# nh273/caro-ai

Measured on AMD Instinct MI355X. Metric: self-play MCTS node-expansions/sec/GPU (Connect4, 200 sims/move); 1->8 GPU scaling, higher is better.
Workload: dtype f32

## Files before the change

caro_ai_amd/_lib.py:

```python
import ctypes as C
import os

_HERE = os.path.dirname(os.path.abspath(__file__))
LIB_PATH = os.path.join(_HERE, "libcaro_hip.so")
if os.environ.get("CARO_HIP_LIB"):
    LIB_PATH = os.environ["CARO_HIP_LIB"]

GAME_CONNECT4, GAME_MNK, GAME_CARO = 0, 1, 2
RESIGNED = -2


class CaroError(RuntimeError):
    pass


class CaroConfig(C.Structure):
    _fields_ = [
        ("game_kind", C.c_int32), ("n", C.c_int32), ("k", C.c_int32), ("n_games", C.c_int32),
        ("n_stores", C.c_int32), ("n_nets", C.c_int32), ("max_batch", C.c_int32), ("node_cap", C.c_int32),
        ("steps_before_tau_0", C.c_int32), ("first_player_mode", C.c_int32),
        ("c_puct", C.c_float), ("alpha", C.c_double), ("explore", C.c_double),
        ("seed", C.c_uint64), ("uid_base", C.c_uint64), ("uid_stride", C.c_uint64),
        ("device_id", C.c_int32), ("evict", C.c_int32), ("stagger", C.c_int32), ("stagger_recycle", C.c_int32),
        ("games_limit", C.c_int64),
# ... 73 lines not shown
    "caro_stream_destroy": (C.c_int, [_P]),
    "caro_search_batch": (C.c_int, [_P, _P, _P, C.c_int, C.c_int, _P, _P, _P, _P, _P, _P]),
    "caro_search_move": (C.c_int, [_P, _P, _P, C.c_int, C.c_int] + [_P] * 10),
    "caro_net_forward_pair": (C.c_int, [_P, _P, _P, _P, C.c_int64, _P, _P, _P]),
    "caro_net_forward_pair_at": (C.c_int, [_P, _P, _P, _P, C.c_int64, C.c_int64, _P, _P, _P]),
    "caro_net_forward_slots": (C.c_int, [_P, _P, _P, _P, _P, C.c_int, C.c_int, _P, _P, _P]),
    "caro_net_forward_slot_list": (C.c_int, [_P, _P, _P, _P, _P, _P, C.c_int, C.c_int, _P, _P, _P]),
    "caro_net_create_hash": (C.c_int, [C.c_int, C.c_int, C.c_int, C.c_uint64, C.c_int, _P]),
    "caro_net_create_hash_grain": (C.c_int, [C.c_int, C.c_int, C.c_int, C.c_uint64, C.c_int, C.c_int, _P]),
    "caro_net_forward_stamped": (C.c_int, [_P, _P, _P, C.c_int, C.c_int64, _P, _P, _P, _P]),
    "caro_net_debug_stamps": (C.c_int, [_P, _P]),
    "caro_get_descent": (C.c_int, [_P, C.c_int, C.c_int, _P, _P, _P, _P, _P, _P]),
    "caro_select_cancel": (C.c_int, [_P]),
    "caro_expand_backup": (C.c_int, [_P, _P, _P, _P]),
    "caro_policy": (C.c_int, [_P, _P, _P, _P]),
    "caro_step": (C.c_int, [_P, _P, _P, _P, _P, _P]),
    "caro_drain_tuples": (C.c_int, [_P, C.c_int64, _P, _P, _P, _P, _P, C.c_int, _P, _P, _P]),
    "caro_drain_tuples_begin": (C.c_int, [_P, C.c_int64, _P, _P, _P, _P, _P, C.c_int, _P]),
    "caro_drain_tuples_end": (C.c_int, [_P, _P, _P]),
    "caro_search_staggered": (C.c_int, [_P, _P, _P, C.c_int, C.c_int, _P, _P, _P, _P, _P]),
    "caro_drain_parked_begin": (C.c_int, [_P, C.c_int64, _P, _P, _P, _P, _P, _P]),
    "caro_engine_set_resign": (C.c_int, [_P, C.c_double, C.c_double]),
    "caro_drain_tuples_begin_q": (C.c_int, [_P, C.c_int64, _P, _P, _P, _P, _P, C.c_int, _P, _P]),
    "caro_drain_parked_begin_q": (C.c_int, [_P, C.c_int64, _P, _P, _P, _P, _P, _P, _P]),
    "caro_engine_set_playout_cap": (C.c_int, [_P, C.c_double, C.c_int]),
    "caro_drain_tuples_begin_x": (C.c_int, [_P, C.c_int64, _P, _P, _P, _P, _P, C.c_int, _P, _P, _P]),
    "caro_drain_parked_begin_x": (C.c_int, [_P, C.c_int64, _P, _P, _P, _P, _P, _P, _P, _P]),
    "caro_engine_set_early_stop": (C.c_int, [_P, C.c_int]),
    "caro_engine_set_openings": (C.c_int, [_P, C.c_int]),
    "caro_engine_set_forced_playouts": (C.c_int, [_P, C.c_double]),
    "caro_forced_stats": (C.c_int, [_P, _P, _P]),
    "caro_engine_set_kernel_form": (C.c_int, [_P, C.c_int]),
    "caro_engine_kernel_form": (C.c_int, [_P]),
    "caro_engine_set_fpu": (C.c_int, [_P, C.c_double, C.c_double]),
    "caro_host_fpu_level": (C.c_int, [C.c_int, C.c_int, _P, _P, _P, _P, _P, _P, _P, C.c_float, C.c_double, C.c_float,
                                      C.c_double, _P]),
    "caro_engine_set_virtual_loss": (C.c_int, [_P, C.c_int]),
    "caro_host_vl_level": (C.c_int, [C.c_int, C.c_int, _P, _P, _P, _P, _P, _P, _P, C.c_float, C.c_double, _P, C.c_int, _P]),
    "caro_engine_set_temperature": (C.c_int, [_P, C.c_double, C.c_double, C.c_int]),
    "caro_host_temperature": (C.c_int, [C.c_int, _P, C.c_double, _P]),
    "caro_host_forced_root": (C.c_int, [C.c_int, _P, _P, _P, _P, C.c_double, C.c_double, _P]),
    "caro_host_forced_prune": (C.c_int, [C.c_int, _P, _P, _P, C.c_float, C.c_double, _P]),
    "caro_drain_tuples_begin_ex": (C.c_int, [_P, C.c_int64, _P, _P, _P, _P, _P, C.c_int, C.POINTER(CaroDrainExtra), _P]),
    "caro_drain_parked_begin_ex": (C.c_int, [_P, C.c_int64, _P, _P, _P, _P, _P, C.POINTER(CaroDrainExtra), _P]),
    "caro_pool_open": (C.c_int, [_P, C.c_int64, _P, _P, _P, _P]),
    "caro_pool_set": (C.c_int, [_P, C.c_int64, _P, _P, _P, _P, _P]),
    "caro_pool_select": (C.c_int, [_P, C.c_int64, _P, _P]),
    "caro_pool_hold": (C.c_int, [_P, _P]),
    "caro_pool_level": (C.c_int, [_P, C.c_int64, _P, _P, _P, _P]),
    "caro_pool_select_budget": (C.c_int, [_P, C.c_int64, _P, _P, _P]),
    "caro_principal_lines": (C.c_int, [_P, C.c_int64, _P, C.c_int, C.c_int, C.c_int] + [_P] * 11),
    "caro_host_line_heads": (C.c_int, [C.c_int, _P, C.c_int, _P]),
    "caro_counters": (C.c_int, [_P, _P, _P]),
    "caro_live_games": (C.c_int, [_P, _P, _P]),
    "caro_pending_leaves": (C.c_int, [_P, _P, _P]),
    "caro_debug_stamps": (C.c_int, [_P, C.c_int]),
    "caro_debug_read": (C.c_int, [_P, _P, C.c_int64, _P]),
    "caro_debug_sqrt_check": (C.c_int, [C.c_uint32, _P]),
    "caro_profile_enable": (C.c_int, [_P, C.c_int]),
    "caro_profile_read": (C.c_int, [_P, _P, _P, C.c_int]),
    "caro_profile_begin": (C.c_int, [_P, C.c_int, _P]),
    "caro_profile_end": (None, [_P, C.c_int, _P]),
    "caro_tree_sizes": (C.c_int, [_P, _P, _P]),
    "caro_tree_live": (C.c_int, [_P, _P, _P]),
    "caro_lookup_nodes": (C.c_int, [_P, C.c_int64] + [_P] * 10),
    "caro_get_roots": (C.c_int, [_P] * 6),
# ... 33 lines not shown
```

caro_ai_amd/csrc/caro_engine.hip:

```cpp
#include <hip/hip_runtime.h>

#include <cstddef>
#include <cstdio>
#include <cstdlib>
#include <cstring>
#include <string>
#include <type_traits>
#include <vector>

#include "../../include/caro_hip.h"
#include "../../include/caro_noise.h"
#include "caro_rules.h"
#include "caro_variants.h"

namespace caro {

constexpr uint32_t NSTRONG = 1u << 30;
constexpr uint32_t NMASK = NSTRONG - 1u;
constexpr int ST_DROPPED = 0, ST_TERMINAL = 1, ST_LEAF = 2;
constexpr int MAXB = 64;
constexpr int DONE_HELD = 3;

enum Counter { C_SIMS, C_LEVELS, C_EXPANSIONS, C_TERMINALS, C_DROPPED, C_OVERFLOW, C_PLIES, C_FINISHED, C_N };

// ... 2615 lines not shown
    s_t[tid] += a;
    s_g[tid] += b;
    __syncthreads();
  }
  long long ot = s_t[tid] - ct;
  int og = s_g[tid] - cg;
  __shared__ long long s_tot;
  __shared__ int s_totg;
  if (tid == 0) { s_tot = 0; s_totg = 0; }
  __syncthreads();
  for (int g = lo; g < hi; ++g) {
    int sel = 0;
    if (v.done[g] == 1) {
      if (ot + v.ply[g] <= cap) {
        sel = 1;
        v.dr_off[g] = (int)ot;
        v.dr_gidx[g] = og;
        atomicMax((unsigned long long*)&s_tot, (unsigned long long)(ot + v.ply[g]));
        atomicMax(&s_totg, og + 1);
      }
      ot += v.ply[g];
      og += 1;
    }
    v.dr_sel[g] = sel;
  }
  __syncthreads();
  if (tid == 0) {
    v.dr_tot[0] = s_tot;
    v.dr_tot[1] = s_totg;
  }
}

template <class GEO>
__global__ void k_drain_copy(View v, uint64_t* __restrict__ states, int32_t* __restrict__ players,
                             double* __restrict__ pi, int32_t* __restrict__ z, int64_t* __restrict__ games,
                             double* __restrict__ root_q, uint8_t* __restrict__ full, uint16_t* __restrict__ mbs,
                             int16_t* __restrict__ open, int recycle) {
  constexpr int KW = GEO::KW;
  const int g = blockIdx.x;
  if (!v.dr_sel[g]) return;
  const int n = v.ply[g];
  const int off = v.dr_off[g];
  const int r = v.final_r[g];
  const uint64_t uid0 = v.uid[g];
  const int16_t made0 = open ? v.open_made[g] : (int16_t)0;
  for (int idx = threadIdx.x; idx < n * v.A; idx += blockDim.x) {
    const int j = idx / v.A, a = idx % v.A;
    const int plyi = n - 1 - j;
    pi[((size_t)off + j) * v.A + a] = v.h_pi[((size_t)g * v.maxply + plyi) * v.A + a];
  }
  for (int j = threadIdx.x; j < n; j += blockDim.x) {
    const int plyi = n - 1 - j;
    const size_t hi = (size_t)g * v.maxply + plyi;
    for (int w = 0; w < KW; ++w) states[((size_t)off + j) * KW + w] = v.h_key[hi * KW + w];
    players[off + j] = v.h_player[hi];
    z[off + j] = (j & 1) ? -r : r;
    if (root_q) root_q[off + j] = v.h_q[hi];
    if (full) full[off + j] = v.h_full[hi];
    if (mbs) mbs[off + j] = v.h_mb[hi];
    if (open) open[off + j] = made0;
  }
  if (threadIdx.x == 0 && games) {
    int64_t* rec = games + (size_t)v.dr_gidx[g] * 4;
    rec[0] = (int64_t)uid0;
    rec[1] = v.first[g];
    rec[2] = v.result[g];
    rec[3] = v.step[g];
  }
  __syncthreads();
  if (recycle && game_wanted(v, g, uid0 + v.uid_stride)) {
    reset_game<GEO>(v, g, uid0 + v.uid_stride, -1);
  } else if (threadIdx.x == 0) {
    v.done[g] = 2;
  }
}

__global__ void k_sum_counters(View v) {
  __shared__ unsigned long long s[256];
  for (int c = 0; c < C_N; ++c) {
    unsigned long long acc = 0;
    for (int g = threadIdx.x; g < v.G; g += blockDim.x) acc += v.counters[(size_t)g * C_N + c];
    s[threadIdx.x] = acc;
    __syncthreads();
    for (int d = 128; d > 0; d >>= 1) {
      if (threadIdx.x < d) s[threadIdx.x] += s[threadIdx.x + d];
      __syncthreads();
    }
    if (threadIdx.x == 0) v.counters_sum[c] = s[0];
    __syncthreads();
  }
}

__global__ void k_sum_forced(View v) {
  __shared__ unsigned long long s[256];
  for (int c = 0; c < 4; ++c) {
    unsigned long long acc = 0;
    for (int g = threadIdx.x; g < v.G; g += blockDim.x) acc += v.fp_ctr[(size_t)g * 4 + c];
    s[threadIdx.x] = acc;
    __syncthreads();
    for (int d = 128; d > 0; d >>= 1) {
      if (threadIdx.x < d) s[threadIdx.x] += s[threadIdx.x + d];
      __syncthreads();
    }
    if (threadIdx.x == 0) v.fp_sum[c] = s[0];
    __syncthreads();
  }
// ... 296 lines not shown
__global__ void k_noise(uint64_t seed, long long M, int A, double alpha, const uint64_t* uid, const uint32_t* ply,
                        const uint32_t* sim, double* out) {
  constexpr int LPD = GEO::LPD, APL = GEO::APL;
  const int grp = threadIdx.x / LPD, l = threadIdx.x % LPD;
  const long long m = (long long)blockIdx.x * (blockDim.x / LPD) + grp;
  const long long mm = m < M ? m : M - 1;
  const uint64_t key = caro_noise_key(seed, uid[mm], ply[mm], sim[mm]);
  double nz[APL];
  __shared__ double s_mail[APL > 1 ? 2 * GEO::AP : 1];
  noise_group<LPD, APL>(key, l, A, alpha, nz, s_mail);
  if (m < M)
    for (int j = 0; j < APL; ++j) {
      const int a = l * APL + j;
      if (a < A) out[(size_t)m * A + a] = nz[j];
    }
}

}

using namespace caro;

static thread_local std::string g_err;
static int fail(int code, const std::string& msg) {
  g_err = msg;
  return code;
}
#define HIPCHK(x)                                                                                  \
  do {                                                                                             \
    hipError_t e_ = (x);                                                                           \
    if (e_ != hipSuccess)                                                                          \
      return fail(CARO_E_HIP, std::string(#x) + ": " + hipGetErrorString(e_));                     \
  } while (0)

struct caro_engine {
  caro_config cfg{};
  Variant var = V_BAD;
  View v{};
  std::vector<void*> allocs;
  int32_t* pinned = nullptr;
  int64_t* pinned64 = nullptr;
  int32_t* scratch = nullptr;
  int32_t* live = nullptr;
  int select_pending = 0;
  int drain_pending = 0;
  int ls_mid = 0;
  int ls_forced = 0;
  int stag_batch = 0;
  hipEvent_t drain_ev = nullptr;
  int prof_on = 0;
  int prof_gate = 1;
  uint64_t prof_ctr = 0;
  uint64_t prof_cal = 0;
  int32_t* rows = nullptr;
  int rows_par = 0;
  int fused_ok = 1;
  int force_full = 0;
  int32_t* pool_host = nullptr;
  std::vector<hipEvent_t> ev;
  std::vector<int> ev_kind;
  size_t ev_used = 0;
  double prof_ms[8] = {};
  long long prof_n[8] = {};
};

static bool tree_lean(const caro_engine* h) {
  const View& v = h->v;
  return !h->force_full && !v.q_on && !v.cap_on && !v.es_on && !v.open_made && !v.fp_on && !v.fpu_on && !v.vl_n && !v.temp_on && !v.lv_on && v.n_stores == 1 && !v.dbg;
}
static bool tree_vl(const caro_engine* h, int batch) { return h->v.vl_n > 0 && batch > 1; }
enum TreeForm { FORM_LEAN, FORM_FULL, FORM_VL };
static TreeForm opening_form(const caro_engine* h, int batch, bool one_wave) {
  if (one_wave && tree_lean(h)) return FORM_LEAN;
  return tree_vl(h, batch) ? FORM_VL : FORM_FULL;
}
static TreeForm closing_form(const caro_engine* h, bool one_wave) { return one_wave && tree_lean(h) ? FORM_LEAN : FORM_FULL; }
#define TREE_FORMS3(form, EXPR)                            \
  switch (form) {                                          \
    case FORM_LEAN: { using OPT = TreeLean; EXPR; } break; \
    case FORM_VL: { using OPT = TreeVl; EXPR; } break;     \
    default: { using OPT = TreeFull; EXPR; } break;        \
  }
#define TREE_FORMS2(form, EXPR)                            \
  if ((form) == FORM_VL) { using OPT = TreeVl; EXPR; }     \
  else { using OPT = TreeFull; EXPR; }

enum : unsigned { R_LEVELS = 1, R_STAG = 2, R_SELECT = 4, R_DRAIN = 8 };
static int guard(const caro_engine* h, const char* who, unsigned what,
                 const char* stag_tail = "use caro_search_staggered / caro_drain_parked_begin") {
  const auto no = [who](const char* text, const char* tail = "") { return fail(CARO_E_STATE, std::string(who) + text + tail); };
// ... 233 lines not shown
  int rc = 0;
#define DA(p, n) if ((rc = dalloc(h, &p, (n))) != 0) { caro_engine_destroy(h); return rc; }
  DA(v.tbl, T);
  DA(v.node_key, T * v.ntab * v.tstride * KW);
  DA(v.edges, T * v.etab * v.tstride * 4 * AP);
  DA(v.n_nodes, T);
  DA(v.n_created, T);
  DA(v.root, G * KW);
  DA(v.player, G); DA(v.ply, G); DA(v.step, G); DA(v.uid, G); DA(v.done, G); DA(v.result, G); DA(v.final_r, G);
  DA(v.first, G);
  DA(v.h_key, G * v.maxply * KW);
  DA(v.h_player, G * v.maxply);
  DA(v.h_pi, G * v.maxply * v.A);
  DA(v.path_rec, G * v.maxB * v.maxd);
  DA(v.d_rec, G * v.maxB);
  DA(v.d_key, G * v.maxB * KW);
  DA(v.g_nleaf, G); DA(v.g_off, G); DA(v.g_tree, G); DA(v.g_class, G); DA(v.g_pack, G);
  DA(v.slot_list, 2 * G * v.maxB);
  DA(v.leaf_count, 4);
  DA(v.counters, G * C_N);
  DA(v.counters_sum, C_N);
  DA(v.dr_off, G); DA(v.dr_gidx, G); DA(v.dr_sel, G); DA(v.dr_tot, 2);
  DA(h->scratch, (size_t)v.maxd + 8);
  DA(h->live, 1);
  DA(h->rows, 8);
  if (cfg->stagger > 0) {
    DA(v.lm, G); DA(v.pend, G); DA(v.wait, G); DA(v.dirty, T);
    DA(v.pk_flag, G); DA(v.pk_ply, G); DA(v.pk_final_r, G); DA(v.pk_first, G); DA(v.pk_result, G); DA(v.pk_step, G);
    DA(v.pk_uid, G);
    DA(v.handed, 1);
    DA(v.ph_key, G * v.maxply * KW);
    DA(v.ph_player, G * v.maxply);
    DA(v.ph_pi, G * v.maxply * v.A);
  }
#undef DA
  HIPCHK(hipHostMalloc((void**)&h->pinned, 64, hipHostMallocDefault));
  HIPCHK(hipHostMalloc((void**)&h->pinned64, 128, hipHostMallocDefault));
  *out = h;
  rc = fresh_state(h, nullptr);
  if (rc) { caro_engine_destroy(h); *out = nullptr; return rc; }
  HIPCHK(hipDeviceSynchronize());
  return 0;
}

int caro_engine_restart(caro_engine* h, const caro_config* cfg, void* stream) {
  if (!h || !cfg) return fail(CARO_E_INVAL, "null argument");
  const caro_config& o = h->cfg;
  if (cfg->game_kind != o.game_kind || cfg->n != o.n || cfg->k != o.k || cfg->n_games != o.n_games ||
      cfg->n_stores != o.n_stores || cfg->n_nets != o.n_nets || cfg->max_batch != o.max_batch ||
      cfg->node_cap != o.node_cap || (cfg->evict != 0) != (o.evict != 0) || cfg->device_id != o.device_id ||
      (cfg->stagger > 0) != (o.stagger > 0))
    return fail(CARO_E_INVAL, "caro_engine_restart: the configuration differs from the engine's in a field that shapes its "
                              "memory (game, n_games, n_stores, n_nets, max_batch, node_cap, evict, device, staggered or not)");
  if (cfg->stagger < 0) return fail(CARO_E_INVAL, "stagger must be >= 0");
  if (int rc = guard(h, "caro_engine_restart", R_DRAIN)) return rc;
  if (int rc = guard(h, "caro_engine_restart", R_SELECT)) return rc;
  HIPCHK(hipSetDevice(o.device_id));
  h->cfg = *cfg;
  apply_run_params(h, cfg);
  return fresh_state(h, (hipStream_t)stream);
}

int caro_engine_set_resign(caro_engine* h, double threshold, double playthrough) {
  if (!h) return fail(CARO_E_INVAL, "null engine");
  if (!(threshold >= -1.0 && threshold <= 1.0)) return fail(CARO_E_INVAL, "resign threshold must be in [-1, 1]");
  if (!(playthrough >= 0.0 && playthrough <= 1.0)) return fail(CARO_E_INVAL, "resign playthrough must be in [0, 1]");
  View& v = h->v;
  if (!v.q_on) {
    HIPCHK(hipSetDevice(h->cfg.device_id));
    const size_t n = (size_t)v.G * v.maxply;
// ... 557 lines not shown

int caro_drain_parked_begin(caro_engine* h, int64_t cap, uint64_t* states, int32_t* players, double* pi, int32_t* z,
                            int64_t* games, void* stream) {
  return caro_drain_parked_begin_q(h, cap, states, players, pi, z, games, nullptr, stream);
}
int caro_drain_parked_begin_q(caro_engine* h, int64_t cap, uint64_t* states, int32_t* players, double* pi, int32_t* z,
                              int64_t* games, double* root_q, void* stream) {
  return caro_drain_parked_begin_x(h, cap, states, players, pi, z, games, root_q, nullptr, stream);
}
int caro_drain_parked_begin_x(caro_engine* h, int64_t cap, uint64_t* states, int32_t* players, double* pi, int32_t* z,
                              int64_t* games, double* root_q, uint8_t* full, void* stream) {
  caro_drain_extra ex = {(uint32_t)sizeof(caro_drain_extra), root_q, full, nullptr, nullptr};
  return caro_drain_parked_begin_ex(h, cap, states, players, pi, z, games, &ex, stream);
}
static int drain_extra(const caro_engine* h, const char* who, const caro_drain_extra* in, caro_drain_extra* out) {
  *out = caro_drain_extra{(uint32_t)sizeof(caro_drain_extra), nullptr, nullptr, nullptr, nullptr};
  if (!in) return 0;
  if (in->size < offsetof(caro_drain_extra, root_q_dev)) return fail(CARO_E_INVAL, "caro_drain_extra.size is not set");
  if (in->size >= offsetof(caro_drain_extra, root_q_dev) + sizeof(double*)) out->root_q_dev = in->root_q_dev;
  if (in->size >= offsetof(caro_drain_extra, full_dev) + sizeof(uint8_t*)) out->full_dev = in->full_dev;
  if (in->size >= offsetof(caro_drain_extra, minibatches_dev) + sizeof(uint16_t*)) out->minibatches_dev = in->minibatches_dev;
  if (in->size >= offsetof(caro_drain_extra, open_dev) + sizeof(int16_t*)) out->open_dev = in->open_dev;
  const std::string w(who);
  if (out->open_dev && !h->v.open_made) return fail(CARO_E_STATE, w + "_ex: open_dev before caro_engine_set_openings (no opening counts recorded)");
  if (out->minibatches_dev && !h->v.es_on) return fail(CARO_E_STATE, w + "_ex: minibatches_dev before caro_engine_set_early_stop (no minibatch counts recorded)");
  if (out->root_q_dev && !h->v.q_on) return fail(CARO_E_STATE, w + "_q before caro_engine_set_resign (no root Q recorded)");
  if (out->full_dev && !h->v.cap_on) return fail(CARO_E_STATE, w + "_x before caro_engine_set_playout_cap (no ply classes recorded)");
  return 0;
}
static int drain_rows(caro_engine* h, const char* who, const View& dv, int64_t cap, uint64_t* states, int32_t* players,
                      double* pi, int32_t* z, int64_t* games, const caro_drain_extra& ex, int recycle, hipStream_t st) {
  if (h->drain_pending) return fail(CARO_E_STATE, std::string(who) + " twice without caro_drain_tuples_end");
  if (!h->drain_ev) HIPCHK(hipEventCreateWithFlags(&h->drain_ev, hipEventDisableTiming));
  hipLaunchKernelGGL(k_drain_scan, dim3(1), dim3(1024), 0, st, dv, (long long)cap);
  DISPATCH(h->var, hipLaunchKernelGGL(k_drain_copy<GEO>, dim3(dv.G), dim3(256), 0, st, dv, states, players, pi, z, games,
                                      ex.root_q_dev, ex.full_dev, ex.minibatches_dev, ex.open_dev, recycle));
  return 0;
}
static int drain_totals(caro_engine* h, hipStream_t st) {
  HIPCHK(hipGetLastError());
  HIPCHK(hipMemcpyAsync(h->pinned64 + 8, h->v.dr_tot, 2 * sizeof(int64_t), hipMemcpyDeviceToHost, st));
  HIPCHK(hipEventRecord(h->drain_ev, st));
  h->drain_pending = 1;
  return 0;
}
int caro_drain_parked_begin_ex(caro_engine* h, int64_t cap, uint64_t* states, int32_t* players, double* pi, int32_t* z,
                               int64_t* games, const caro_drain_extra* extra, void* stream) {
  if (!h || !states || !players || !pi || !z) return fail(CARO_E_INVAL, "null argument");
  caro_drain_extra ex;
  if (int rc = drain_extra(h, "caro_drain_parked_begin", extra, &ex)) return rc;
  if (!h->v.stag_S) return fail(CARO_E_STATE, "the engine was not created in staggered mode (caro_config.stagger)");
  hipStream_t st = (hipStream_t)stream;
  View pv = h->v;
  pv.done = h->v.pk_flag; pv.ply = h->v.pk_ply; pv.final_r = h->v.pk_final_r; pv.first = h->v.pk_first;
  pv.result = h->v.pk_result; pv.step = h->v.pk_step; pv.uid = h->v.pk_uid;
  pv.h_key = h->v.ph_key; pv.h_player = h->v.ph_player; pv.h_pi = h->v.ph_pi; pv.h_q = h->v.ph_q;
  pv.h_full = h->v.ph_full;
  pv.h_mb = h->v.ph_mb;
  pv.open_made = h->v.pk_open;
  if (int rc = drain_rows(h, "caro_drain_parked_begin", pv, cap, states, players, pi, z, games, ex, 0, st)) return rc;
  if (h->v.stag_pool)
    DISPATCH(h->var, hipLaunchKernelGGL(k_stag_assign<GEO>, dim3(1), dim3(1024), 0, st, h->v));
  DISPATCH(h->var, hipLaunchKernelGGL(k_stag_clean<GEO>, dim3(h->v.G * h->v.n_stores), dim3(256), 0, st, h->v));
  return drain_totals(h, st);
}

int caro_policy(caro_engine* h, double* pi, int32_t* counts, void* stream) {
  if (!h) return fail(CARO_E_INVAL, "null engine");
  DISPATCH(h->var, hipLaunchKernelGGL(k_policy<GEO>, dim3(h->v.G), dim3(64), 0, (hipStream_t)stream, h->v, pi, counts));
  HIPCHK(hipGetLastError());
  return 0;
}

int caro_step(caro_engine* h, const double* uniforms, int32_t* actions, int32_t* done, int32_t* result, void* stream) {
  if (!h) return fail(CARO_E_INVAL, "null engine");
  if (int rc = guard(h, "caro_step", R_STAG | R_SELECT)) return rc;
  const int p0 = prof_begin(h, PK_STEP, (hipStream_t)stream);
  DISPATCH(h->var, hipLaunchKernelGGL(k_step<GEO>, dim3(h->v.G), dim3(64), 0, (hipStream_t)stream, h->v, uniforms,
                                      actions, done, result));
  prof_end(h, p0, (hipStream_t)stream);
  h->ls_mid = 0;
  h->ls_forced = 0;
  if (h->cfg.evict)
    DISPATCH(h->var, hipLaunchKernelGGL(k_evict<GEO>, dim3(h->v.G), dim3(256), 0, (hipStream_t)stream, h->v));
  HIPCHK(hipGetLastError());
  return 0;
}

int caro_drain_tuples_begin(caro_engine* h, int64_t cap, uint64_t* states, int32_t* players, double* pi, int32_t* z,
                            int64_t* games, int recycle, void* stream) {
  return caro_drain_tuples_begin_q(h, cap, states, players, pi, z, games, recycle, nullptr, stream);
}
// ... 50 lines not shown
  *counts_dev = h->v.leaf_count;
  return 0;
}

int caro_stream_create_partition(int device_id, int part, int nparts, void** stream_out) {
  if (!stream_out || nparts < 1 || part < 0 || part >= nparts) return fail(CARO_E_INVAL, "bad partition");
  HIPCHK(hipSetDevice(device_id));
  hipDeviceProp_t prop;
  HIPCHK(hipGetDeviceProperties(&prop, device_id));
  const int ncu = prop.multiProcessorCount;
  const int words = (ncu + 31) / 32;
  std::vector<uint32_t> mask(words, 0u);
  const int lo = (int)((long long)ncu * part / nparts), hi = (int)((long long)ncu * (part + 1) / nparts);
  for (int c = lo; c < hi; ++c) mask[c >> 5] |= 1u << (c & 31);
  hipStream_t st = nullptr;
  HIPCHK(hipExtStreamCreateWithCUMask(&st, (uint32_t)words, mask.data()));
  *stream_out = (void*)st;
  return 0;
}
int caro_stream_destroy(void* stream) {
  if (stream) HIPCHK(hipStreamDestroy((hipStream_t)stream));
  return 0;
}

int caro_engine_set_kernel_form(caro_engine* h, int form) {
  if (!h) return fail(CARO_E_INVAL, "null engine");
  if (form != 0 && form != 1) return fail(CARO_E_INVAL, "kernel form must be 0 (automatic) or 1 (always the full form)");
  h->force_full = form;
  return 0;
}
int caro_engine_kernel_form(const caro_engine* h) {
  if (!h) return fail(CARO_E_INVAL, "null engine");
  return tree_lean(h) ? 0 : 1;
}

int caro_debug_stamps(caro_engine* h, int on) {
  if (!h) return fail(CARO_E_INVAL, "null engine");
  if (on && !h->v.dbg) {
    void* q = nullptr;
    HIPCHK(hipMalloc(&q, (size_t)h->v.G * 16 * sizeof(unsigned long long)));
    HIPCHK(hipMemset(q, 0, (size_t)h->v.G * 16 * sizeof(unsigned long long)));
    h->allocs.push_back(q);
    h->v.dbg = (unsigned long long*)q;
  } else if (!on) {
    h->v.dbg = nullptr;
  }
  return 0;
}
int caro_debug_read(caro_engine* h, uint64_t* out_host, int64_t n_u64, void* stream) {
  if (!h || !out_host || !h->v.dbg) return fail(CARO_E_INVAL, "no stamp buffer");
  if (n_u64 > (int64_t)h->v.G * 16) n_u64 = (int64_t)h->v.G * 16;
  HIPCHK(hipStreamSynchronize((hipStream_t)stream));
  HIPCHK(hipMemcpy(out_host, h->v.dbg, n_u64 * sizeof(uint64_t), hipMemcpyDeviceToHost));
  return 0;
}

int caro_debug_sqrt_check(uint32_t n_max, uint64_t* bad_host) {
  if (!bad_host || n_max > (1u << 24)) return fail(CARO_E_INVAL, "bad argument");
  unsigned long long* bad = nullptr;
  HIPCHK(hipMalloc(&bad, sizeof(unsigned long long)));
  HIPCHK(hipMemset(bad, 0, sizeof(unsigned long long)));
  hipLaunchKernelGGL(k_sqrt_check, dim3(1024), dim3(256), 0, (hipStream_t) nullptr, n_max, bad);
  HIPCHK(hipGetLastError());
  HIPCHK(hipMemcpy(bad_host, bad, sizeof(unsigned long long), hipMemcpyDeviceToHost));
  HIPCHK(hipFree(bad));
  return 0;
// ... 146 lines not shown
```

caro_ai_amd/engine.py:

```python
import ctypes as C

import numpy as np
import torch

from caro_ai_amd import _lib
from caro_ai_amd import early_stop
from caro_ai_amd import forced_playouts as forced_playouts_mod
from caro_ai_amd import fpu as fpu_mod
from caro_ai_amd import openings as openings_mod
from caro_ai_amd import selfplay_options
from caro_ai_amd import temperature as temperature_mod
from caro_ai_amd import virtual_loss as virtual_loss_mod
from caro_ai_amd import config as cfg

COUNTER_NAMES = ["sims", "levels", "expansions", "terminals", "dropped", "overflows", "plies", "finished"]


HIP_NET_MODES = {"hip": "f32", "hipw": "f32w", "hipw1": "f32w1", "hipw2": "f32w2", "hipx3": "bf16x3"}

def lanes_per_descent(game):
    A = game.action_space
    return 8 if A == 7 else 16 if A <= 16 else 32 if A <= 32 else 64


def staggered_geometry(game, batch, evict=False):
    t = int(batch) * lanes_per_descent(game)
    return t >= 64 and t % 64 == 0 and (t > 64 or not evict)


def _ptr(t):
    return C.c_void_p(t.data_ptr()) if t is not None else None


def torch_evaluator(net, form="gemm"):
    from caro_ai_amd.lib.model import GemmNet, Net
    net.eval()
    if form == "gemm" and isinstance(net, Net):
        dev = next(net.parameters()).device
        net = GemmNet(net).to(dev).eval()

    @torch.no_grad()
    def fn(planes):
        logits, values = net(planes)
        return torch.softmax(logits.float(), dim=1).contiguous(), values.float().reshape(-1).contiguous()

    return fn


class SelfPlayEngine:
    VIEW_LIMIT_BYTES = 16 << 20
    DEFAULT_CAP_LIMIT = 1 << 16
    EVICT_DEFAULT_CAP = 1 << 13

    def __init__(self, game, n_games, net1=None, net2=None, evaluators=None, n_stores=1, max_batch=None,
                 node_cap=None, steps_before_tau_0=cfg.STEPS_BEFORE_TAU_0, first_player_mode=2,
                 c_puct=cfg.C_PUCT, alpha=cfg.ALPHA, explore=cfg.EXPLORE, seed=0, uid_base=0, uid_stride=None,
                 device="cuda:0", searches_hint=cfg.MCTS_SEARCHES, inference="hipw", evict=False, stagger=False,
                 stagger_recycle=True, games_limit=0):
        if not torch.cuda.is_available():
            raise _lib.CaroError("SelfPlayEngine needs a GPU (torch.cuda.is_available() is False); "
                                 "there is no CPU fallback")
        self.L = _lib.load()
        self.game = game
        self.device = torch.device(device)
        self.G = int(n_games)
        self.A = game.action_space
        self.KW = game.key_words
        self.obs_shape = tuple(game.obs_shape)
        self.HW = self.obs_shape[1] * self.obs_shape[2]
        self.max_batch = int(max_batch or cfg.MCTS_BATCH_SIZE)
        if evaluators is None:
            nets = [net1] if net2 is None or net2 is net1 else [net1, net2]
            if inference in HIP_NET_MODES:
                from caro_ai_amd.net_hip import HipNet
                mode = HIP_NET_MODES[inference]
                evaluators = [HipNet(n, str(self.device), mode=mode) for n in nets]
            else:
                evaluators = [torch_evaluator(n.to(self.device), form=inference) for n in nets]
        self.evaluators = list(evaluators)
        self.async_net = all(getattr(e, "device_counts", False) for e in self.evaluators)
        self.n_nets = len(self.evaluators)
        assert self.n_nets in (1, 2)
        if node_cap is None:
            node_cap = self.default_node_cap(searches_hint, self.max_batch, self.HW, evict)
        c = _lib.CaroConfig()
        c.game_kind, c.n, c.k = game.kind, game.n, game.k
        c.n_games, c.n_stores, c.n_nets = self.G, n_stores, self.n_nets
        c.max_batch, c.node_cap = self.max_batch, int(node_cap)
        c.steps_before_tau_0, c.first_player_mode = steps_before_tau_0, first_player_mode
        c.c_puct, c.alpha, c.explore = c_puct, alpha, explore
        c.seed, c.uid_base = seed, uid_base
        c.uid_stride = uid_stride if uid_stride is not None else self.G
        c.device_id = self.device.index or 0
        c.evict = 1 if evict else 0
        self.stagger = bool(stagger)
        self.stag_S = int(searches_hint)
        if self.stagger and not self.async_net:
            raise _lib.CaroError("stagger=True needs device-side evaluators (the fused HIP net or HashNet)")
        c.stagger = self.stag_S if self.stagger else 0
        c.stagger_recycle = int(stagger_recycle)
        c.games_limit = int(games_limit or 0)
        self.stagger_recycle = bool(stagger_recycle)
        self.cfg = c
        self.n_stores = n_stores
        torch.cuda.set_device(self.device)
        h = C.c_void_p()
        _lib.check(self.L.caro_engine_create(C.byref(c), C.byref(h)))
        self.h = h
        rows = self.G * self.max_batch
        self.planes = torch.zeros((rows,) + self.obs_shape, dtype=torch.float32, device=self.device)
        self.leaf_keys = torch.zeros((rows, self.KW), dtype=torch.int64, device=self.device)
        self._probs = torch.zeros((rows, self.A), dtype=torch.float32, device=self.device)
        self._values = torch.zeros(rows, dtype=torch.float32, device=self.device)
        self._counts = (C.c_int32 * 2)()
        cd = C.c_void_p()
        _lib.check(self.L.caro_leaf_counts_dev(self.h, C.byref(cd)))
        self._counts_dev = cd
        self.maxply = self.HW
        self._row_bytes = 8 * self.KW + 8 * self.A + 8
        self.net_rows = 0
        self.net_calls = 0
        self._prof = False
        self._drain_open = False
        self.resign = None
        self.playout_cap = None
        self.early_stop = None
        self.openings = None
        self.forced_playouts = None
        self.fpu = None
        self.virtual_loss = None
        self.temperature = None

    @classmethod
    def default_node_cap(cls, searches, max_batch, cells, evict=False):
        bound = int(searches) * int(max_batch) * int(cells) + 64
        if bound <= cls.DEFAULT_CAP_LIMIT:
            return bound
        if not evict:
            raise _lib.CaroError(
                "SelfPlayEngine: %d searches x %d descents x %d cells needs up to %d nodes per tree, more than the %d a "
                "default tree holds; pass evict=True (unreachable nodes are dropped after every move, result-neutral: "
# ... 69 lines not shown
            self._row_bytes += 2
        if self.openings is not None or m > 0:
            self.openings = m

    def set_forced_playouts(self, k):
        kf = forced_playouts_mod.check_k(k)
        _lib.check(self.L.caro_engine_set_forced_playouts(self.h, kf))
        if self.forced_playouts is not None or kf > 0:
            self.forced_playouts = kf

    def set_fpu(self, reduction, root_reduction=None):
        r = fpu_mod.check_reduction(reduction)
        rr = r if root_reduction is None else fpu_mod.check_reduction(root_reduction, "root reduction")
        _lib.check(self.L.caro_engine_set_fpu(self.h, r, rr))
        if self.fpu is not None or r > 0 or rr > 0:
            self.fpu = (r, rr)

    def set_virtual_loss(self, n):
        nv = virtual_loss_mod.check_n(n)
        _lib.check(self.L.caro_engine_set_virtual_loss(self.h, nv))
        if self.virtual_loss is not None or nv > 0:
            self.virtual_loss = nv

    def set_temperature(self, early=1.0, late=0.0, visit_targets=False):
        triple = temperature_mod.check_triple(early, late, visit_targets)
        _lib.check(self.L.caro_engine_set_temperature(self.h, triple[0], triple[1], int(triple[2])))
        self.temperature = triple if temperature_mod.is_on(triple) else None

    def set_kernel_form(self, form):
        _lib.check(self.L.caro_engine_set_kernel_form(self.h, int(form)))

    def kernel_form(self):
        form = self.L.caro_engine_kernel_form(self.h)
        if form < 0:
            _lib.check(form)
        return form

    def __del__(self):
        try:
            self.close()
        except Exception:
            pass

    def _stream(self):
        return C.c_void_p(torch.cuda.current_stream(self.device).cuda_stream)

    def reset(self, first_players=None):
        fp = None
        if first_players is not None:
            fp = torch.as_tensor(first_players, dtype=torch.int32).to(self.device).contiguous()
        _lib.check(self.L.caro_reset_games(self.h, _ptr(fp), self._stream()))
        if fp is not None:
            torch.cuda.current_stream(self.device).synchronize()

    def set_roots(self, states, players):
        keys = torch.from_numpy(self.game.to_keys(states).view(np.int64)).to(self.device)
        pl = torch.as_tensor(players, dtype=torch.int32).to(self.device)
        _lib.check(self.L.caro_set_roots(self.h, _ptr(keys), _ptr(pl), self._stream()))
        torch.cuda.current_stream(self.device).synchronize()

    def _i32(self, values):
        return torch.as_tensor(np.asarray(values, dtype=np.int32).reshape(-1)).to(self.device)

    def pool_open(self, slots, uids, first_players):
        g, fp = self._i32(slots), self._i32(first_players)
        uid = torch.as_tensor(np.asarray(uids, dtype=np.uint64).reshape(-1).view(np.int64)).to(self.device)
# ... 476 lines not shown
```

include/caro_hip.h:

```cpp
#ifndef CARO_HIP_H
#define CARO_HIP_H

#include <stdint.h>

#ifdef __cplusplus
extern "C" {
#endif

#define CARO_GAME_CONNECT4 0
#define CARO_GAME_MNK 1
#define CARO_GAME_CARO 2

#define CARO_E_INVAL (-22)
#define CARO_E_NOMEM (-12)
#define CARO_E_HIP (-5)
#define CARO_E_NODEV (-19)
#define CARO_E_STATE (-71)

#define CARO_RESIGNED (-2)

typedef struct caro_engine caro_engine;

typedef struct caro_config {
  int32_t game_kind;
// ... 103 lines not shown
                              int32_t* z_dev, int64_t* games_dev, double* root_q_dev, uint8_t* full_dev, void* stream);

int caro_engine_set_early_stop(caro_engine* h, int min_minibatches);

int caro_engine_set_openings(caro_engine* h, int max_plies);

int caro_engine_set_forced_playouts(caro_engine* h, double k);
int caro_forced_stats(caro_engine* h, int64_t out[4], void* stream);

int caro_engine_set_fpu(caro_engine* h, double reduction, double root_reduction);

int caro_engine_set_virtual_loss(caro_engine* h, int n_vl);

int caro_engine_set_temperature(caro_engine* h, double tau_early, double tau_late, int visit_targets);

int caro_pool_open(caro_engine* h, int64_t M, const int32_t* games_dev, const uint64_t* uid_dev,
                   const int32_t* first_player_dev, void* stream);
int caro_pool_set(caro_engine* h, int64_t M, const int32_t* games_dev, const uint64_t* keys_dev,
                  const int32_t* players_dev, const int32_t* ply_dev, void* stream);
int caro_pool_select(caro_engine* h, int64_t M, const int32_t* games_dev, void* stream);
int caro_pool_hold(caro_engine* h, void* stream);
int caro_pool_level(caro_engine* h, int64_t M, const int32_t* games_dev, const int32_t* net_dev, const double* tau_dev,
                    void* stream);
int caro_pool_select_budget(caro_engine* h, int64_t M, const int32_t* games_dev, const int32_t* budget_dev, void* stream);

int caro_principal_lines(caro_engine* h, int64_t M, const int32_t* games_dev, int store, int top, int depth,
                         int32_t* n_lines_dev, int32_t* root_visits_dev, int32_t* len_dev, int32_t* end_dev,
                         int32_t* move_dev, int32_t* N_dev, float* W_dev, float* Q_dev, float* P_dev,
                         int32_t* strong_dev, void* stream);
int caro_host_line_heads(int A, const int32_t* N, int top, int32_t* heads_out);

int caro_engine_set_kernel_form(caro_engine* h, int form);
int caro_engine_kernel_form(const caro_engine* h);

typedef struct caro_drain_extra {
  uint32_t size;
  double* root_q_dev;
  uint8_t* full_dev;
  uint16_t* minibatches_dev;
  int16_t* open_dev;
} caro_drain_extra;
int caro_drain_tuples_begin_ex(caro_engine* h, int64_t cap, uint64_t* states_dev, int32_t* players_dev, double* pi_dev,
                               int32_t* z_dev, int64_t* games_dev, int recycle, const caro_drain_extra* extra,
                               void* stream);
int caro_drain_parked_begin_ex(caro_engine* h, int64_t cap, uint64_t* states_dev, int32_t* players_dev, double* pi_dev,
                               int32_t* z_dev, int64_t* games_dev, const caro_drain_extra* extra, void* stream);

int caro_counters(caro_engine* h, int64_t counters[8], void* stream);
int caro_profile_enable(caro_engine* h, int on);
int caro_profile_begin(caro_engine* h, int kind, void* stream);
void caro_profile_end(caro_engine* h, int slot, void* stream);
int caro_profile_read(caro_engine* h, double ms[8], int64_t launches[8], int reset);
int caro_debug_stamps(caro_engine* h, int on);
int caro_debug_read(caro_engine* h, uint64_t* out_host, int64_t n_u64, void* stream);
int caro_debug_sqrt_check(uint32_t n_max, uint64_t* bad_host);
int caro_live_games(caro_engine* h, int32_t* live, void* stream);
int caro_pending_leaves(caro_engine* h, int32_t* pending, void* stream);

int caro_tree_sizes(caro_engine* h, int32_t* out_dev, void* stream);
int caro_tree_live(caro_engine* h, int32_t* out_dev, void* stream);
int caro_lookup_nodes(caro_engine* h, int64_t M, const int32_t* game_dev, const int32_t* store_dev,
                      const uint64_t* keys_dev, int32_t* found_dev, int32_t* N_dev, float* W_dev, float* Q_dev,
                      float* P_dev, int32_t* strong_dev, void* stream);
int caro_get_roots(caro_engine* h, uint64_t* keys_dev, int32_t* players_dev, int32_t* ply_dev, uint64_t* uid_dev,
                   void* stream);
int caro_poke_nodes(caro_engine* h, int64_t M, const int32_t* game_dev, const int32_t* store_dev,
// ... 74 lines not shown
```

Measured before the change: 8.620 million.

## Fuse drain scan, table clean and totals copy into two kernels

Adds a new drain path, on by default, that uses a parallel per-wave scan select kernel, which also builds a list of dirty tables in a second block. A single rows kernel then both clears the dirty hash-table keys and copies game tuples. The totals are written straight to coherent pinned host memory from the device, which removes a separate D2H memcpy and the old scan/copy/clean launch sequence. The cost is that pinned64 now uses coherent host memory, and stag_assign is reordered ahead of the drain in the parked path.

Measured after the change: 8.649 million, median of 6. No clear change (+0.3%).

```diff
diff --git a/caro_ai_amd/_lib.py b/caro_ai_amd/_lib.py
--- a/caro_ai_amd/_lib.py
+++ b/caro_ai_amd/_lib.py
@@ -129,6 +129,8 @@
     "caro_forced_stats": (C.c_int, [_P, _P, _P]),
     "caro_engine_set_kernel_form": (C.c_int, [_P, C.c_int]),
     "caro_engine_kernel_form": (C.c_int, [_P]),
+    "caro_engine_set_drain_form": (C.c_int, [_P, C.c_int]),
+    "caro_engine_drain_form": (C.c_int, [_P]),
     "caro_engine_set_fpu": (C.c_int, [_P, C.c_double, C.c_double]),
     "caro_host_fpu_level": (C.c_int, [C.c_int, C.c_int, _P, _P, _P, _P, _P, _P, _P, C.c_float, C.c_double, C.c_float,
                                       C.c_double, _P]),
diff --git a/caro_ai_amd/csrc/caro_engine.hip b/caro_ai_amd/csrc/caro_engine.hip
--- a/caro_ai_amd/csrc/caro_engine.hip
+++ b/caro_ai_amd/csrc/caro_engine.hip
@@ -2671,12 +2671,12 @@
 }
 
 template <class GEO>
-__global__ void k_drain_copy(View v, uint64_t* __restrict__ states, int32_t* __restrict__ players,
-                             double* __restrict__ pi, int32_t* __restrict__ z, int64_t* __restrict__ games,
-                             double* __restrict__ root_q, uint8_t* __restrict__ full, uint16_t* __restrict__ mbs,
-                             int16_t* __restrict__ open, int recycle) {
+__device__ __forceinline__ void drain_copy_game(const View& v, int g, uint64_t* __restrict__ states,
+                                                int32_t* __restrict__ players, double* __restrict__ pi,
+                                                int32_t* __restrict__ z, int64_t* __restrict__ games,
+                                                double* __restrict__ root_q, uint8_t* __restrict__ full,
+                                                uint16_t* __restrict__ mbs, int16_t* __restrict__ open, int recycle) {
   constexpr int KW = GEO::KW;
-  const int g = blockIdx.x;
   if (!v.dr_sel[g]) return;
   const int n = v.ply[g];
   const int off = v.dr_off[g];
@@ -2711,6 +2711,113 @@
     reset_game<GEO>(v, g, uid0 + v.uid_stride, -1);
   } else if (threadIdx.x == 0) {
     v.done[g] = 2;
+  }
+}
+
+template <class GEO>
+__global__ void k_drain_copy(View v, uint64_t* __restrict__ states, int32_t* __restrict__ players,
+                             double* __restrict__ pi, int32_t* __restrict__ z, int64_t* __restrict__ games,
+                             double* __restrict__ root_q, uint8_t* __restrict__ full, uint16_t* __restrict__ mbs,
+                             int16_t* __restrict__ open, int recycle) {
+  drain_copy_game<GEO>(v, blockIdx.x, states, players, pi, z, games, root_q, full, mbs, open, recycle);
+}
+
+struct DrainAux {
+  int32_t* clist;
+  int32_t* nclean;
+  int64_t* tot_host;
+};
+
+__global__ void __launch_bounds__(1024) k_drain_select(View v, long long cap, DrainAux ax, int T) {
+  const int tid = threadIdx.x, lane = tid & 63, w = tid >> 6;
+  if (blockIdx.x == 1) {
+    __shared__ int s_n;
+    if (tid == 0) s_n = 0;
+    __syncthreads();
+    for (int t = tid; t < T; t += 1024)
+      if (v.dirty[t]) {
+        ax.clist[atomicAdd(&s_n, 1)] = t * 2 + (1 - v.tbl[t]);
+        v.dirty[t] = 0;
+      }
+    __syncthreads();
+    if (tid == 0) ax.nclean[0] = s_n;
+    return;
+  }
+  __shared__ long long s_wt[16];
+  __shared__ int s_wg[16];
+  __shared__ long long s_tot;
+  __shared__ int s_totg;
+  const int chunk = (v.G + 1023) / 1024;
+  const int lo = min(v.G, tid * chunk), hi = min(v.G, lo + chunk);
+  long long ct = 0;
+  int cg = 0;
+  for (int g = lo; g < hi; ++g)
+    if (v.done[g] == 1) { ct += v.ply[g]; cg += 1; }
+  long long it = ct;
+  int ig = cg;
+  for (int d = 1; d < 64; d <<= 1) {
+    const long long a = __shfl_up(it, d);
+    const int b = __shfl_up(ig, d);
+    if (lane >= d) { it += a; ig += b; }
+  }
+  if (lane == 63) { s_wt[w] = it; s_wg[w] = ig; }
+  if (tid == 0) { s_tot = 0; s_totg = 0; }
+  __syncthreads();
+  long long ot = it - ct;
+  int og = ig - cg;
+  for (int k = 0; k < w; ++k) { ot += s_wt[k]; og += s_wg[k]; }
+  for (int g = lo; g < hi; ++g) {
+    int sel = 0;
+    if (v.done[g] == 1) {
+      const int n = v.ply[g];
+      if (ot + n <= cap) {
+        sel = 1;
+        v.dr_off[g] = (int)ot;
+        v.dr_gidx[g] = og;
+        atomicMax((unsigned long long*)&s_tot, (unsigned long long)(ot + n));
+        atomicMax(&s_totg, og + 1);
+      }
+      ot += n;
+      og += 1;
+    }
+    v.dr_sel[g] = sel;
+  }
+  __syncthreads();
+  if (tid == 0) {
+    v.dr_tot[0] = s_tot;
+    v.dr_tot[1] = s_totg;
+  }
+}
+
+template <class GEO>
+__global__ void __launch_bounds__(256) k_drain_rows(View v, uint64_t* __restrict__ states, int32_t* __restrict__ players,
+                                                    double* __restrict__ pi, int32_t* __restrict__ z,
+                                                    int64_t* __restrict__ games, double* __restrict__ root_q,
+                                                    uint8_t* __restrict__ full, uint16_t* __restrict__ mbs,
+                                                    int16_t* __restrict__ open, int recycle, DrainAux ax,
+                                                    int nclean_blocks) {
+  constexpr int KW = GEO::KW;
+  if ((int)blockIdx.x >= nclean_blocks) {
+    if ((int)blockIdx.x == nclean_blocks && threadIdx.x == 0) {
+      ax.tot_host[0] = v.dr_tot[0];
+      ax.tot_host[1] = v.dr_tot[1];
+      __threadfence_system();
+    }
+    drain_copy_game<GEO>(v, (int)blockIdx.x - nclean_blocks, states, players, pi, z, games, root_q, full, mbs, open, recycle);
+    return;
+  }
+  const int sh = __ffs(v.hcap) - 2;
+  const size_t units = ((size_t)ax.nclean[0] << sh) * KW;
+  const bool wide = ((v.tstride * KW) & 1) == 0;
+  for (size_t u = (size_t)blockIdx.x * 256 + threadIdx.x; u < units; u += (size_t)nclean_blocks * 256) {
+    const size_t i = (u / KW) >> sh;
+    uint64_t* keys = v.node_key + (size_t)ax.clist[i] * v.tstride * KW + (u - ((i << sh) * KW)) * 2;
+    if (wide) {
+      *reinterpret_cast<ulonglong2*>(keys) = make_ulonglong2(EMPTY_KEY, EMPTY_KEY);
+    } else {
+      keys[0] = EMPTY_KEY;
+      keys[1] = EMPTY_KEY;
+    }
   }
 }
 
@@ -3073,6 +3180,11 @@
       return fail(CARO_E_HIP, std::string(#x) + ": " + hipGetErrorString(e_));                     \
   } while (0)
 
+static const int g_drain_form_env = [] {
+  const char* e = getenv("CARO_DRAIN_FORM");
+  return e && e[0] == '0' && !e[1] ? 0 : 1;
+}();
+
 struct caro_engine {
   caro_config cfg{};
   Variant var = V_BAD;
@@ -3096,6 +3208,8 @@
   int rows_par = 0;
   int fused_ok = 1;
   int force_full = 0;
+  int drain_form = g_drain_form_env;
+  DrainAux dax{};
   int32_t* pool_host = nullptr;
   std::vector<hipEvent_t> ev;
   std::vector<int> ev_kind;
@@ -3395,10 +3509,12 @@
     DA(v.ph_key, G * v.maxply * KW);
     DA(v.ph_player, G * v.maxply);
     DA(v.ph_pi, G * v.maxply * v.A);
+    DA(h->dax.clist, T); DA(h->dax.nclean, 1);
   }
 #undef DA
   HIPCHK(hipHostMalloc((void**)&h->pinned, 64, hipHostMallocDefault));
-  HIPCHK(hipHostMalloc((void**)&h->pinned64, 128, hipHostMallocDefault));
+  HIPCHK(hipHostMalloc((void**)&h->pinned64, 128, hipHostMallocCoherent));
+  HIPCHK(hipHostGetDevicePointer((void**)&h->dax.tot_host, h->pinned64 + 8, 0));
   *out = h;
   rc = fresh_state(h, nullptr);
   if (rc) { caro_engine_destroy(h); *out = nullptr; return rc; }
@@ -4022,6 +4138,16 @@
                       double* pi, int32_t* z, int64_t* games, const caro_drain_extra& ex, int recycle, hipStream_t st) {
   if (h->drain_pending) return fail(CARO_E_STATE, std::string(who) + " twice without caro_drain_tuples_end");
   if (!h->drain_ev) HIPCHK(hipEventCreateWithFlags(&h->drain_ev, hipEventDisableTiming));
+  if (h->drain_form == 1) {
+    const int T = dv.G * dv.n_stores;
+    const size_t all = dv.dirty ? (size_t)T * (dv.hcap / 2) * variant_kw(h->var) : 0;
+    const int nclean = (int)std::min<size_t>(256, (all + 2047) / 2048);
+    hipLaunchKernelGGL(k_drain_select, dim3(dv.dirty ? 2 : 1), dim3(1024), 0, st, dv, (long long)cap, h->dax, T);
+    DISPATCH(h->var, hipLaunchKernelGGL(k_drain_rows<GEO>, dim3(nclean + dv.G), dim3(256), 0, st, dv, states, players, pi,
+                                        z, games, ex.root_q_dev, ex.full_dev, ex.minibatches_dev, ex.open_dev, recycle,
+                                        h->dax, nclean));
+    return 0;
+  }
   hipLaunchKernelGGL(k_drain_scan, dim3(1), dim3(1024), 0, st, dv, (long long)cap);
   DISPATCH(h->var, hipLaunchKernelGGL(k_drain_copy<GEO>, dim3(dv.G), dim3(256), 0, st, dv, states, players, pi, z, games,
                                       ex.root_q_dev, ex.full_dev, ex.minibatches_dev, ex.open_dev, recycle));
@@ -4029,7 +4155,8 @@
 }
 static int drain_totals(caro_engine* h, hipStream_t st) {
   HIPCHK(hipGetLastError());
-  HIPCHK(hipMemcpyAsync(h->pinned64 + 8, h->v.dr_tot, 2 * sizeof(int64_t), hipMemcpyDeviceToHost, st));
+  if (h->drain_form != 1)
+    HIPCHK(hipMemcpyAsync(h->pinned64 + 8, h->v.dr_tot, 2 * sizeof(int64_t), hipMemcpyDeviceToHost, st));
   HIPCHK(hipEventRecord(h->drain_ev, st));
   h->drain_pending = 1;
   return 0;
@@ -4048,6 +4175,13 @@
   pv.h_full = h->v.ph_full;
   pv.h_mb = h->v.ph_mb;
   pv.open_made = h->v.pk_open;
+  if (h->drain_form == 1) {
+    if (h->drain_pending) return fail(CARO_E_STATE, "caro_drain_parked_begin twice without caro_drain_tuples_end");
+    if (h->v.stag_pool)
+      DISPATCH(h->var, hipLaunchKernelGGL(k_stag_assign<GEO>, dim3(1), dim3(1024), 0, st, h->v));
+    if (int rc = drain_rows(h, "caro_drain_parked_begin", pv, cap, states, players, pi, z, games, ex, 0, st)) return rc;
+    return drain_totals(h, st);
+  }
   if (int rc = drain_rows(h, "caro_drain_parked_begin", pv, cap, states, players, pi, z, games, ex, 0, st)) return rc;
   if (h->v.stag_pool)
     DISPATCH(h->var, hipLaunchKernelGGL(k_stag_assign<GEO>, dim3(1), dim3(1024), 0, st, h->v));
@@ -4164,6 +4298,18 @@
 int caro_engine_kernel_form(const caro_engine* h) {
   if (!h) return fail(CARO_E_INVAL, "null engine");
   return tree_lean(h) ? 0 : 1;
+}
+
+int caro_engine_set_drain_form(caro_engine* h, int form) {
+  if (!h) return fail(CARO_E_INVAL, "null engine");
+  if (form != 0 && form != 1) return fail(CARO_E_INVAL, "drain form must be 0 (scan, copy, clean, copy of the totals) or 1 (select, rows)");
+  if (int rc = guard(h, "caro_engine_set_drain_form", R_DRAIN)) return rc;
+  h->drain_form = form;
+  return 0;
+}
+int caro_engine_drain_form(const caro_engine* h) {
+  if (!h) return fail(CARO_E_INVAL, "null engine");
+  return h->drain_form;
 }
 
 int caro_debug_stamps(caro_engine* h, int on) {
diff --git a/caro_ai_amd/engine.py b/caro_ai_amd/engine.py
--- a/caro_ai_amd/engine.py
+++ b/caro_ai_amd/engine.py
@@ -56,7 +56,7 @@
                  node_cap=None, steps_before_tau_0=cfg.STEPS_BEFORE_TAU_0, first_player_mode=2,
                  c_puct=cfg.C_PUCT, alpha=cfg.ALPHA, explore=cfg.EXPLORE, seed=0, uid_base=0, uid_stride=None,
                  device="cuda:0", searches_hint=cfg.MCTS_SEARCHES, inference="hipw", evict=False, stagger=False,
-                 stagger_recycle=True, games_limit=0):
+                 stagger_recycle=True, games_limit=0, drain_form=None):
         if not torch.cuda.is_available():
             raise _lib.CaroError("SelfPlayEngine needs a GPU (torch.cuda.is_available() is False); "
                                  "there is no CPU fallback")
@@ -107,6 +107,8 @@
         h = C.c_void_p()
         _lib.check(self.L.caro_engine_create(C.byref(c), C.byref(h)))
         self.h = h
+        if drain_form is not None:
+            self.set_drain_form(drain_form)
         rows = self.G * self.max_batch
         self.planes = torch.zeros((rows,) + self.obs_shape, dtype=torch.float32, device=self.device)
         self.leaf_keys = torch.zeros((rows, self.KW), dtype=torch.int64, device=self.device)
@@ -242,6 +244,15 @@
 
     def kernel_form(self):
         form = self.L.caro_engine_kernel_form(self.h)
+        if form < 0:
+            _lib.check(form)
+        return form
+
+    def set_drain_form(self, form):
+        _lib.check(self.L.caro_engine_set_drain_form(self.h, int(form)))
+
+    def drain_form(self):
+        form = self.L.caro_engine_drain_form(self.h)
         if form < 0:
             _lib.check(form)
         return form
diff --git a/include/caro_hip.h b/include/caro_hip.h
--- a/include/caro_hip.h
+++ b/include/caro_hip.h
@@ -159,6 +159,9 @@
 
 int caro_engine_set_kernel_form(caro_engine* h, int form);
 int caro_engine_kernel_form(const caro_engine* h);
+
+int caro_engine_set_drain_form(caro_engine* h, int form);
+int caro_engine_drain_form(const caro_engine* h);
 
 typedef struct caro_drain_extra {
   uint32_t size;
```
